# paulffm/Continuous-Time-Diffusion-Models-for-Discrete-Data

Measured on AMD Instinct MI355X. Metric: tau-leaping sample-steps/s, higher is better.
Workload: dtype bf16; 1 GPU; MNIST tauLDR U-Net TauL step (config_tauUnet_mnist: D=784, S=256, 1000-step grid); batch_per_gpu=256, global_batch=256, D=784, S=256, parallelism=sample-sharded x1, no collective in the loop

## Files before the change

continuous-time-diffusion-models-for-discrete-data_amd/csrc/unet_resblock_kernels.hip:

```cpp
#include "row_tile.hpp"
#include "../../include/ctdd_unet.h"

namespace ctdd {
namespace {

constexpr int RB_THREADS = 256, RB_N = 192, RB_PST = 20, RB_MAXC = 384;

struct RbLds {
  int raw, slab, part, red, scale, total;
  int rsA, rs2, prows;
};
__host__ __device__ inline RbLds rb_layout(int H, int W, int C) {
  RbLds L;
  L.rsA = C * 2 + 32;
  L.rs2 = RB_N * 2 + 32;
  L.prows = (H + 2) * (W + 2);
  const int slabA = L.prows * L.rsA, slab2 = L.prows * L.rs2;
  L.raw = 0;
  L.slab = H * W * L.rsA;
  L.part = L.slab + (slabA > slab2 ? slabA : slab2);
  L.red = L.part + RB_THREADS * RB_PST * 4;
  L.scale = L.red + 2 * RB_MAXC * 8;
  L.total = L.scale + 2 * RB_MAXC * 4;
  return L;
// ... 128 lines not shown
  auto step = [&](u32x4 (&slot)[3][2], bf16x8 (&xf)[NPT][2], bf16x8 (&xnext)[NPT][2], int ci, auto guard) {
    constexpr bool GUARD = decltype(guard)::value;
    if (GUARD && ci >= nchunks) return;
    xload(xnext, ci + 1);
#pragma unroll
    for (int s = 0; s < 2; ++s)
#pragma unroll
      for (int t = 0; t < 3; ++t)
#pragma unroll
        for (int pt = 0; pt < NPT; ++pt)
          acc[t][pt] = __builtin_amdgcn_mfma_f32_16x16x32_bf16(__builtin_bit_cast(bf16x8, slot[t][s]), xf[pt][s], acc[t][pt], 0, 0, 0);
    if (!GUARD || ci + PD < nchunks) wload(slot, ci + PD);
  };
  static_assert(PD % 2 == 0, "the two pixel-fragment buffers alternate inside a group");
  bf16x8 xq[2][NPT][2];
  xload(xq[0], 0);
  int ci0 = 0;
  for (; ci0 + 2 * PD <= nchunks; ci0 += PD) {
#pragma unroll
    for (int u = 0; u < PD; ++u) step(wr[u], xq[u & 1], xq[(u + 1) & 1], ci0 + u, std::false_type{});
  }
  for (; ci0 < nchunks; ci0 += PD) {
#pragma unroll
    for (int u = 0; u < PD; ++u) step(wr[u], xq[u & 1], xq[(u + 1) & 1], ci0 + u, std::true_type{});
  }
}

template <int NPT>
__global__ __launch_bounds__(RB_THREADS, 1) void k_resblock_small(const ctdd_resblock_args a) {
  extern __shared__ __attribute__((aligned(16))) unsigned char sm[];
  constexpr int PD = 6;
  const int t = threadIdx.x, b = blockIdx.x;
  const int H = a.H, W = a.W, HW = H * W, C = a.C1 + a.C2, Wp = W + 2;
  const RbLds L = rb_layout(H, W, C);
  const int lane = t & 63, wv = t >> 6, lj = lane & 15, lq = lane >> 4;

  const int K1 = 9 * C, K2 = 9 * RB_N + (a.skip ? C : 0);
  const unsigned short* w1p = (const unsigned short*)a.w1 + (size_t)wv * (K1 / 64) * 3072 + lane * 8;
  const unsigned short* w2p = (const unsigned short*)a.w2 + (size_t)wv * (K2 / 64) * 3072 + lane * 8;
  u32x4 wr[PD][3][2];

  {
    const int noct = C >> 3, nvec = HW * noct;
    const unsigned short* s1 = (const unsigned short*)a.s1_bf16 + (size_t)b * HW * a.C1;
    const unsigned short* s2 = (const unsigned short*)a.s2_bf16 + (size_t)b * HW * a.C2;
    constexpr int MAXV = 12;
    u32x4 u[MAXV];
#pragma unroll
    for (int k = 0; k < MAXV; ++k) {
      const int v = t + k * RB_THREADS, p = v / noct, c0 = (v - p * noct) * 8;
      const unsigned short* src = c0 < a.C1 ? s1 + (size_t)p * a.C1 + c0 : s2 + (size_t)p * a.C2 + (c0 - a.C1);
      u[k] = v < nvec ? *(const u32x4*)src : (u32x4){0u, 0u, 0u, 0u};
    }
    rb_wprologue<PD>(wr, w1p);
#pragma unroll
    for (int k = 0; k < MAXV; ++k) {
      const int v = t + k * RB_THREADS, p = v / noct, c0 = (v - p * noct) * 8;
      if (v < nvec) *(u32x4*)(sm + L.raw + p * L.rsA + c0 * 2) = u[k];
    }
    const int nz = (L.part - L.slab) >> 4;
    for (int v = t; v < nz; v += RB_THREADS) *(uint4*)(sm + L.slab + v * 16) = make_uint4(0, 0, 0, 0);
    __syncthreads();
    rb_groupnorm(sm, L, L.raw, L.rsA, false, L.slab, L.rsA, HW, W, Wp, C, a.G1, a.gamma1, a.beta1, a.eps1);
  }

  int pix[NPT], prow[NPT], b3[NPT], b1[NPT];
#pragma unroll
  for (int pt = 0; pt < NPT; ++pt) {
    if constexpr (NPT == 1) {
      const int pe = lj < HW ? lj : HW - 1;
      pix[pt] = lj < HW ? lj : -1;
      prow[pt] = rb_prow(pe, W, Wp);
      b1[pt] = L.raw + pe * L.rsA + lq * 16;
    } else {
      const RbPix q = rb_tile_pixel(pt, lj, H, W);
      pix[pt] = q.ok ? q.p : -1;
      prow[pt] = q.row;
      b1[pt] = L.raw + q.p * L.rsA + lq * 16;
    }
    b3[pt] = L.slab + prow[pt] * L.rsA + lq * 16;
  }
  const int n0 = wv * 48;
  f32x4 acc[3][NPT];
#pragma unroll
  for (int tt = 0; tt < 3; ++tt)
#pragma unroll
    for (int pt = 0; pt < NPT; ++pt) acc[tt][pt] = (f32x4){0.0f, 0.0f, 0.0f, 0.0f};

  rb_gemm<NPT, PD>(acc, wr, w1p, K1 / 64, K1 / 64, C / 64, sm, b3, L.rsA, Wp, b1);
  __syncthreads();
  rb_wprologue<PD>(wr, w2p);
  {
    const int npc = L.rs2 >> 4, nv = L.prows * npc;
    for (int v = t; v < nv; v += RB_THREADS) {
      const int row = v / npc, y = row / Wp, x = row - y * Wp;
      if (y == 0 || y == H + 1 || x == 0 || x == W + 1) *(uint4*)(sm + L.slab + v * 16) = make_uint4(0, 0, 0, 0);
    }
#pragma unroll
    for (int tt = 0; tt < 3; ++tt) {
      const int n = n0 + tt * 16 + lq * 4;
      const float4 bv = *(const float4*)(a.bias1 + n);
      const float4 tb = a.tbias ? *(const float4*)(a.tbias + (size_t)b * a.tb_stride + n) : make_float4(0.0f, 0.0f, 0.0f, 0.0f);
      const float add[4] = {bv.x + tb.x, bv.y + tb.y, bv.z + tb.z, bv.w + tb.w};
#pragma unroll
      for (int pt = 0; pt < NPT; ++pt) {
        if (pix[pt] >= 0) {
          const f32x4 v = acc[tt][pt];
          *(uint2*)(sm + L.slab + prow[pt] * L.rs2 + n * 2) =
              make_uint2(rt_pack2(v[0] + add[0], v[1] + add[1]), rt_pack2(v[2] + add[2], v[3] + add[3]));
        }
        acc[tt][pt] = (f32x4){0.0f, 0.0f, 0.0f, 0.0f};
      }
    }
  }
  __syncthreads();

  rb_groupnorm(sm, L, L.slab, L.rs2, true, L.slab, L.rs2, HW, W, Wp, RB_N, a.G2, a.gamma2, a.beta2, a.eps2);

#pragma unroll
  for (int pt = 0; pt < NPT; ++pt) b3[pt] = L.slab + prow[pt] * L.rs2 + lq * 16;
  rb_gemm<NPT, PD>(acc, wr, w2p, K2 / 64, 9 * RB_N / 64, RB_N / 64, sm, b3, L.rs2, Wp, b1);
  __syncthreads();
#pragma unroll
  for (int tt = 0; tt < 3; ++tt) {
    const int n = n0 + tt * 16 + lq * 4;
    const float4 bv = *(const float4*)(a.bias2 + n);
#pragma unroll
    for (int pt = 0; pt < NPT; ++pt) {
      if (pix[pt] >= 0) {
        const f32x4 v = acc[tt][pt];
        float o[4] = {v[0] + bv.x, v[1] + bv.y, v[2] + bv.z, v[3] + bv.w};
        if (!a.skip) {
          const uint2 r = *(const uint2*)(sm + L.raw + pix[pt] * L.rsA + n * 2);
          o[0] += __uint_as_float(r.x << 16); o[1] += __uint_as_float(r.x & 0xFFFF0000u);
          o[2] += __uint_as_float(r.y << 16); o[3] += __uint_as_float(r.y & 0xFFFF0000u);
        }
        *(uint2*)(sm + L.slab + pix[pt] * L.rs2 + n * 2) = make_uint2(rt_pack2(o[0], o[1]), rt_pack2(o[2], o[3]));
      }
    }
  }
  __syncthreads();
  {
    constexpr int npc = RB_N / 8;
    unsigned short* out = (unsigned short*)a.out_bf16 + (size_t)b * HW * RB_N;
    for (int v = t; v < HW * npc; v += RB_THREADS) {
      const int p = v / npc, c0 = (v - p * npc) * 8;
      *(uint4*)(out + (size_t)p * RB_N + c0) = *(const uint4*)(sm + L.slab + p * L.rs2 + c0 * 2);
    }
  }
}

constexpr int RM_NPT = 14, RM_PITCH = 16, RM_MAXH = 14, RM_MAXCS = 192;
constexpr int RM_RS = RB_N * 2 + 32;

__host__ __device__ inline RbLds rm_layout(int H, int W) {
  RbLds L;
  (void)W;
  L.rsA = L.rs2 = RB_N * 2 + 32;
  L.prows = (H + 2) * RM_PITCH;
  L.raw = L.slab = L.rs2;
  L.part = (L.prows + 2) * L.rs2;
  L.red = L.part + RB_THREADS * RB_PST * 4;
  L.scale = L.red + 2 * RB_MAXC * 8;
  L.total = L.scale + 2 * RB_MAXC * 4;
  return L;
}

__device__ __attribute__((always_inline)) inline void rm_gn1_stats(unsigned char* sm, const RbLds& L, const unsigned short* __restrict__ s1,
                                                                  const unsigned short* __restrict__ s2, int C1, int C2, int HW, int G,
                                                                  const float* __restrict__ gamma, const float* __restrict__ beta, float eps) {
  const int t = threadIdx.x, C = C1 + C2, noct = C >> 3;
  const int npl = RB_THREADS / noct < HW ? RB_THREADS / noct : HW, T = noct * npl;
  const bool act = t < T;
  const int oct = act ? t % noct : 0, pl = act ? t / noct : 0, c0 = oct * 8;
  const bool first = c0 < C1;
  const unsigned short* src = first ? s1 + c0 : s2 + (c0 - C1);
  const int cs = first ? C1 : C2;
  float* part = (float*)(sm + L.part);
  double* red = (double*)(sm + L.red);
  float* scale = (float*)(sm + L.scale);
  float* shift = scale + RB_MAXC;
  float sx[8], sq[8];
#pragma unroll
  for (int j = 0; j < 8; ++j) { sx[j] = 0.0f; sq[j] = 0.0f; }
  if (act) {
#pragma unroll 4
    for (int p = pl; p < HW; p += npl) {
      const u32x4 u = *(const u32x4*)(src + (size_t)p * cs);
#pragma unroll
      for (int j = 0; j < 4; ++j) {
        const float x0 = __uint_as_float(u[j] << 16), x1 = __uint_as_float(u[j] & 0xFFFF0000u);
        sx[2 * j] += x0; sq[2 * j] = fmaf(x0, x0, sq[2 * j]);
        sx[2 * j + 1] += x1; sq[2 * j + 1] = fmaf(x1, x1, sq[2 * j + 1]);
      }
    }
    float4* pt = (float4*)(part + t * RB_PST);
    pt[0] = make_float4(sx[0], sx[1], sx[2], sx[3]); pt[1] = make_float4(sx[4], sx[5], sx[6], sx[7]);
    pt[2] = make_float4(sq[0], sq[1], sq[2], sq[3]); pt[3] = make_float4(sq[4], sq[5], sq[6], sq[7]);
  }
  __syncthreads();
  for (int r = t; r < 2 * C; r += RB_THREADS) {
    const int m = r >= C ? 1 : 0, c = r - m * C;
    const float* pp = part + (c >> 3) * RB_PST + m * 8 + (c & 7);
    double acc = 0.0;
    for (int q = 0; q < npl; ++q) acc += (double)pp[q * noct * RB_PST];
    red[r] = acc;
  }
  __syncthreads();
  const int cg = C / G;
  for (int c = t; c < C; c += RB_THREADS) {
    const int g0 = (c / cg) * cg;
    double s = 0.0, q = 0.0;
    for (int j = g0; j < g0 + cg; ++j) { s += red[j]; q += red[C + j]; }
    const double n = (double)cg * (double)HW;
    const double mean = s / n;
    const double var = fmax(q / n - mean * mean, 0.0);
    const float rstd = (float)(1.0 / sqrt(var + (double)eps));
    scale[c] = rstd * gamma[c];
    shift[c] = beta[c] - (float)mean * rstd * gamma[c];
  }
  __syncthreads();
}

__device__ __attribute__((always_inline)) inline void rm_gn1_apply(unsigned char* sm, const RbLds& L, const unsigned short* __restrict__ src, int cs,
                                                                  int coff, int HW, int W) {
  const int t = threadIdx.x, noct = cs >> 3, npl = RB_THREADS / noct;
  if (t >= noct * npl) return;
  const int oct = t % noct, pl = t / noct;
  const float* scale = (const float*)(sm + L.scale) + coff + oct * 8;
  const float* shift = scale + RB_MAXC;
  const float4 sc0 = *(const float4*)scale, sc1 = *(const float4*)(scale + 4);
  const float4 sh0 = *(const float4*)shift, sh1 = *(const float4*)(shift + 4);
  const f32x2v scv[4] = {{sc0.x, sc0.y}, {sc0.z, sc0.w}, {sc1.x, sc1.y}, {sc1.z, sc1.w}};
  const f32x2v shv[4] = {{sh0.x, sh0.y}, {sh0.z, sh0.w}, {sh1.x, sh1.y}, {sh1.z, sh1.w}};
  const unsigned short* sp = src + oct * 8;
#pragma unroll 4
  for (int p = pl; p < HW; p += npl) {
    const u32x4 u = *(const u32x4*)(sp + (size_t)p * cs);
    unsigned ow[4];
#pragma unroll
    for (int j = 0; j < 4; ++j) {
      const f32x2v x = {__uint_as_float(u[j] << 16), __uint_as_float(u[j] & 0xFFFF0000u)};
      f32x2v y = __builtin_elementwise_fma(x, scv[j], shv[j]);
      const f32x2v z = y * (f32x2v){-1.4426950408889634f, -1.4426950408889634f};
      const f32x2v d = (f32x2v){__builtin_amdgcn_exp2f(z.x), __builtin_amdgcn_exp2f(z.y)} + (f32x2v){1.0f, 1.0f};
      y = y * (f32x2v){__builtin_amdgcn_rcpf(d.x), __builtin_amdgcn_rcpf(d.y)};
      ow[j] = rt_pack2(y.x, y.y);
    }
    *(uint4*)(sm + L.slab + rb_prow(p, W, RM_PITCH) * L.rs2 + oct * 16) = make_uint4(ow[0], ow[1], ow[2], ow[3]);
  }
}

__device__ __attribute__((always_inline)) inline void rm_wprologue(u32x4 (&wr)[2][3][3], const unsigned short* __restrict__ wrow, int nunits) {
#pragma unroll
  for (int u = 0; u < 2; ++u)
    if (u < nunits) rt_wload9(wr[u], wrow, u);
}

template <bool FULL>
__device__ __attribute__((always_inline)) inline void rm_gemm_skip(f32x4 (&acc)[3][RM_NPT], u32x4 (&ws)[2][3], const unsigned short* __restrict__ wrow, int nsk,
                                                                  const unsigned short* __restrict__ s1, const unsigned short* __restrict__ s2,
                                                                  int C1, int C2, int xc, int lq, int H, int W) {
  const int nc1 = C1 >> 5;
  auto gload = [&](bf16x8 (&g)[RM_NPT], int u) {
    const int ue = u < nsk ? u : nsk - 1;
    const bool two = ue >= nc1;
    const unsigned char* base = (const unsigned char*)(two ? s2 : s1);
    const int cs = two ? C2 : C1, cb = (ue - (two ? nc1 : 0)) * 32 + lq * 8;
#pragma unroll
    for (int y = 0; y < RM_NPT; ++y) {
      const int ye = FULL || y < H ? y : H - 1;
      g[y] = *(const bf16x8*)(base + (unsigned)(((ye * W + xc) * cs + cb) * 2));
    }
  };
  auto step = [&](u32x4 (&slot)[3], bf16x8 (&gc)[RM_NPT], bf16x8 (&gn)[RM_NPT], int u, auto guard) {
    constexpr bool GUARD = decltype(guard)::value;
    if (GUARD && u >= nsk) return;
    gload(gn, u + 1);
#pragma unroll
    for (int y = 0; y < RM_NPT; ++y) {
      if (FULL || y < H) {
#pragma unroll
        for (int t = 0; t < 3; ++t)
          acc[t][y] = __builtin_amdgcn_mfma_f32_16x16x32_bf16(__builtin_bit_cast(bf16x8, slot[t]), gc[y], acc[t][y], 0, 0, 0);
      }
    }
    if (!GUARD || u + 2 < nsk) rt_wload3(slot, wrow, u + 2);
    __builtin_amdgcn_sched_barrier(0);
  };
  bf16x8 G[2][RM_NPT];
  gload(G[0], 0);
  __builtin_amdgcn_s_waitcnt(0x0F70);
  int u0 = 0;
  for (; u0 + 4 <= nsk; u0 += 2) {
    step(ws[0], G[0], G[1], u0, std::false_type{});
    step(ws[1], G[1], G[0], u0 + 1, std::false_type{});
  }
  for (; u0 < nsk; u0 += 2) {
    step(ws[0], G[0], G[1], u0, std::true_type{});
    step(ws[1], G[1], G[0], u0 + 1, std::true_type{});
  }
}

template <bool FULL>
__global__ __launch_bounds__(RB_THREADS, 1) void k_resblock_mid(const ctdd_resblock_args a) {
  extern __shared__ __attribute__((aligned(16))) unsigned char sm[];
  constexpr int NPT = RM_NPT;
  const int t = threadIdx.x, b = blockIdx.x;
  const int H = FULL ? RM_NPT : a.H, W = a.W, HW = H * W, C1 = a.C1, C2 = a.C2;
  const RbLds L = rm_layout(H, W);
  const int lane = t & 63, wv = t >> 6, lj = lane & 15, lq = lane >> 4;
  const int nu1a = 3 * (C1 >> 5), nu1b = 3 * (C2 >> 5), nsk = a.skip ? (C1 + C2) >> 5 : 0;
  const unsigned short* w1p = (const unsigned short*)a.w1 + (size_t)wv * (nu1a + nu1b) * RT_UNIT + lane * 8;
  const unsigned short* s1 = (const unsigned short*)a.s1_bf16 + (size_t)b * HW * C1;
  const unsigned short* s2 = (const unsigned short*)a.s2_bf16 + (size_t)b * HW * C2;
  u32x4 wr[2][3][3];

  rm_wprologue(wr, w1p, nu1a);
  for (int v = t; v < (L.part >> 4); v += RB_THREADS) *(uint4*)(sm + v * 16) = make_uint4(0, 0, 0, 0);
  rm_gn1_stats(sm, L, s1, s2, C1, C2, HW, a.G1, a.gamma1, a.beta1, a.eps1);

  const int fb = L.slab + lj * RM_RS + lq * 16;
  const int n0 = wv * 48;
  f32x4 acc[3][NPT];
#pragma unroll
  for (int tt = 0; tt < 3; ++tt)
#pragma unroll
    for (int pt = 0; pt < NPT; ++pt) acc[tt][pt] = (f32x4){0.0f, 0.0f, 0.0f, 0.0f};

  for (int s = 0; s < (C2 ? 2 : 1); ++s) {
    rm_gn1_apply(sm, L, s ? s2 : s1, s ? C2 : C1, s ? C1 : 0, HW, W);
    __syncthreads();
    rt_gemm_rows<FULL, RM_RS, RM_PITCH>(acc, wr, w1p + (size_t)(s ? nu1a : 0) * RT_UNIT, s ? nu1b : nu1a, sm, fb, H);
    __syncthreads();
    if (s == 0 && C2) rm_wprologue(wr, w1p + (size_t)nu1a * RT_UNIT, nu1b);
  }
  const int tw = rt_again(t);
  const unsigned short* w2p = (const unsigned short*)a.w2 + (size_t)(tw >> 6) * (18 * RT_UNIT + nsk * 1536) + (tw & 63) * 8;
  u32x4 ws[2][3];
  if (nsk) {
    rt_wload3(ws[0], w2p + (size_t)18 * RT_UNIT, 0);
    if (nsk > 1) rt_wload3(ws[1], w2p + (size_t)18 * RT_UNIT, 1);
  } else {
    rm_wprologue(wr, w2p, 18);
  }
  const int lj1 = rt_again(lj);
  const bool own1 = lj1 >= 1 && lj1 <= W;
#pragma unroll
  for (int tt = 0; tt < 3; ++tt) {
    const int n = n0 + tt * 16 + lq * 4;
    const float4 bv = *(const float4*)(a.bias1 + n);
    const float4 tb = a.tbias ? *(const float4*)(a.tbias + (size_t)b * a.tb_stride + n) : make_float4(0.0f, 0.0f, 0.0f, 0.0f);
    const float add[4] = {bv.x + tb.x, bv.y + tb.y, bv.z + tb.z, bv.w + tb.w};
#pragma unroll
    for (int y = 0; y < NPT; ++y) {
      if (y < H && own1) {
        const f32x4 v = acc[tt][y];
        *(uint2*)(sm + L.slab + ((y + 1) * RM_PITCH + lj1) * RM_RS + n * 2) =
            make_uint2(rt_pack2(v[0] + add[0], v[1] + add[1]), rt_pack2(v[2] + add[2], v[3] + add[3]));
      }
      acc[tt][y] = (f32x4){0.0f, 0.0f, 0.0f, 0.0f};
    }
  }
  __syncthreads();

  if (nsk) {
    const int ljs = rt_again(lj), xc = ljs < 1 ? 0 : (ljs > W ? W - 1 : ljs - 1);
    rm_gemm_skip<FULL>(acc, ws, w2p + (size_t)18 * RT_UNIT, nsk, s1, s2, C1, C2, xc, lq, H, W);
    rm_wprologue(wr, w2p, 18);
  }

  rb_groupnorm(sm, L, L.slab, L.rs2, true, L.slab, L.rs2, HW, W, RM_PITCH, RB_N, a.G2, a.gamma2, a.beta2, a.eps2);
  rt_gemm_rows<FULL, RM_RS, RM_PITCH>(acc, wr, w2p, 18, sm, fb, H);
  __syncthreads();
  const int lj2 = rt_again(lj);
  const bool own2 = lj2 >= 1 && lj2 <= W;
  const int x2 = own2 ? lj2 - 1 : 0;
#pragma unroll
  for (int tt = 0; tt < 3; ++tt) {
    const int n = n0 + tt * 16 + lq * 4;
    const float4 bv = *(const float4*)(a.bias2 + n);
    uint2 r[NPT] = {};
    if (!a.skip) {
#pragma unroll
      for (int y = 0; y < NPT; ++y) r[y] = *(const uint2*)(s1 + (size_t)((y < H ? y : H - 1) * W + x2) * RB_N + n);
    }
#pragma unroll
    for (int y = 0; y < NPT; ++y) {
      if (y < H && own2) {
        const f32x4 v = acc[tt][y];
        float o[4] = {v[0] + bv.x, v[1] + bv.y, v[2] + bv.z, v[3] + bv.w};
        if (!a.skip) {
          o[0] += __uint_as_float(r[y].x << 16); o[1] += __uint_as_float(r[y].x & 0xFFFF0000u);
          o[2] += __uint_as_float(r[y].y << 16); o[3] += __uint_as_float(r[y].y & 0xFFFF0000u);
        }
        *(uint2*)(sm + L.slab + (y * W + x2) * RM_RS + n * 2) = make_uint2(rt_pack2(o[0], o[1]), rt_pack2(o[2], o[3]));
      }
    }
  }
  __syncthreads();
  {
    constexpr int npc = RB_N / 8;
    unsigned short* out = (unsigned short*)a.out_bf16 + (size_t)b * HW * RB_N;
    for (int v = t; v < HW * npc; v += RB_THREADS) {
      const int p = v / npc, c0 = (v - p * npc) * 8;
      *(uint4*)(out + (size_t)p * RB_N + c0) = *(const uint4*)(sm + L.slab + p * RM_RS + c0 * 2);
    }
  }
}

}
}

using namespace ctdd;

extern "C" int ctdd_unet_resblock_small(const void* args_, int f32, void* stream) {
  CTDD_REQUIRE(args_, CTDD_EINVAL, "ctdd_unet_resblock_small: null arguments");
  const ctdd_resblock_args& a = *(const ctdd_resblock_args*)args_;
  CTDD_REQUIRE(f32 == 0, CTDD_ERANGE, "ctdd_unet_resblock_small: bf16 inference only (the fp32 mode keeps the four launches)");
  const int span = (a.H - 1) * (a.W + 2) + a.W;
  CTDD_REQUIRE(a.B > 0 && a.H > 0 && a.W > 0 && a.W <= 8 && a.H * a.W <= 64 && (a.H * a.W <= 16 || span <= 80), CTDD_ERANGE,
               "ctdd_unet_resblock_small: a sample of %dx%d pixels does not fit the workgroup tile (H*W <= 64, W <= 8, (H-1)(W+2)+W <= 80)", a.H, a.W);
  const int C = a.C1 + a.C2;
  CTDD_REQUIRE(a.N == RB_N && a.C1 > 0 && a.C1 % 64 == 0 && a.C2 >= 0 && a.C2 % 64 == 0 && C <= RB_MAXC, CTDD_ERANGE,
               "ctdd_unet_resblock_small: channel counts off the tile (N=%d, C1=%d, C2=%d; N = 192, sources in multiples of 64, <= 384)", a.N,
               a.C1, a.C2);
  CTDD_REQUIRE(a.G1 > 0 && C % a.G1 == 0 && a.G2 > 0 && RB_N % a.G2 == 0, CTDD_EINVAL, "ctdd_unet_resblock_small: groups do not divide the channels");
  CTDD_REQUIRE(a.skip || (a.C2 == 0 && a.C1 == RB_N), CTDD_EINVAL, "ctdd_unet_resblock_small: a residual block needs C1 == N and one source");
  CTDD_REQUIRE(a.s1_bf16 && (a.C2 == 0 || a.s2_bf16) && a.w1 && a.w2 && a.bias1 && a.bias2 && a.gamma1 && a.beta1 && a.gamma2 && a.beta2 &&
                   a.out_bf16, CTDD_EINVAL, "ctdd_unet_resblock_small: null pointer");
  const RbLds L = rb_layout(a.H, a.W, C);
  CTDD_REQUIRE(L.total <= 160 * 1024, CTDD_ERANGE, "ctdd_unet_resblock_small: LDS image of %d bytes over the 160 KiB budget", L.total);
  hipStream_t st = (hipStream_t)stream;
  static bool attr_done[3][16] = {};
  if (a.H * a.W <= 16) {
    ensure_lds_ceiling((const void*)k_resblock_small<1>, attr_done[0]);
    hipLaunchKernelGGL(k_resblock_small<1>, dim3(a.B), dim3(RB_THREADS), (size_t)L.total, st, a);
  } else if (span > 64) {
    ensure_lds_ceiling((const void*)k_resblock_small<5>, attr_done[2]);
    hipLaunchKernelGGL(k_resblock_small<5>, dim3(a.B), dim3(RB_THREADS), (size_t)L.total, st, a);
  } else {
    ensure_lds_ceiling((const void*)k_resblock_small<4>, attr_done[1]);
    hipLaunchKernelGGL(k_resblock_small<4>, dim3(a.B), dim3(RB_THREADS), (size_t)L.total, st, a);
  }
  return finish_launch("k_resblock_small");
}

extern "C" int ctdd_unet_resblock_mid(const void* args_, int f32, void* stream) {
  CTDD_REQUIRE(args_, CTDD_EINVAL, "ctdd_unet_resblock_mid: null arguments");
  const ctdd_resblock_args& a = *(const ctdd_resblock_args*)args_;
  CTDD_REQUIRE(f32 == 0, CTDD_ERANGE, "ctdd_unet_resblock_mid: bf16 inference only (the fp32 mode keeps the four launches)");
  CTDD_REQUIRE(a.B > 0 && a.H > 0 && a.W > 0 && a.H <= RM_MAXH && a.W <= RM_PITCH - 2, CTDD_ERANGE,
               "ctdd_unet_resblock_mid: a sample of %dx%d pixels does not fit the workgroup tile (H <= 14, W <= 14)", a.H, a.W);
  const int C = a.C1 + a.C2;
  CTDD_REQUIRE(a.N == RB_N && a.C1 > 0 && a.C1 % 32 == 0 && a.C1 <= RM_MAXCS && a.C2 >= 0 && a.C2 % 32 == 0 && a.C2 <= RM_MAXCS, CTDD_ERANGE,
               "ctdd_unet_resblock_mid: channel counts off the tile (N=%d, C1=%d, C2=%d; N = 192, sources in multiples of 32, <= 192 each)", a.N,
               a.C1, a.C2);
  CTDD_REQUIRE(a.G1 > 0 && C % a.G1 == 0 && a.G2 > 0 && RB_N % a.G2 == 0, CTDD_EINVAL, "ctdd_unet_resblock_mid: groups do not divide the channels");
  CTDD_REQUIRE(a.skip || (a.C2 == 0 && a.C1 == RB_N), CTDD_EINVAL, "ctdd_unet_resblock_mid: a residual block needs C1 == N and one source");
  CTDD_REQUIRE(a.s1_bf16 && (a.C2 == 0 || a.s2_bf16) && a.w1 && a.w2 && a.bias1 && a.bias2 && a.gamma1 && a.beta1 && a.gamma2 && a.beta2 &&
                   a.out_bf16, CTDD_EINVAL, "ctdd_unet_resblock_mid: null pointer");
  const RbLds L = rm_layout(a.H, a.W);
  CTDD_REQUIRE(L.total <= 160 * 1024, CTDD_ERANGE, "ctdd_unet_resblock_mid: LDS image of %d bytes over the 160 KiB budget", L.total);
  static bool attr_done[2][16] = {};
  if (a.H == RM_NPT) {
    ensure_lds_ceiling((const void*)k_resblock_mid<true>, attr_done[1]);
    hipLaunchKernelGGL(k_resblock_mid<true>, dim3(a.B), dim3(RB_THREADS), (size_t)L.total, (hipStream_t)stream, a);
  } else {
    ensure_lds_ceiling((const void*)k_resblock_mid<false>, attr_done[0]);
    hipLaunchKernelGGL(k_resblock_mid<false>, dim3(a.B), dim3(RB_THREADS), (size_t)L.total, (hipStream_t)stream, a);
  }
  return finish_launch("k_resblock_mid");
}
```

continuous-time-diffusion-models-for-discrete-data_amd/csrc/unet_rows_kernels.hip:

```cpp
#include "row_tile.hpp"
#include "../../include/ctdd_unet.h"

namespace ctdd {
namespace {

constexpr int CR_N = 96, CR_BAND = 14, CR_PITCH = 32, CR_RS = 224, CR_MAXW = 28, CR_MAXC = 384, CR_PIECE = 96;
constexpr int CR_SLAB = ((CR_BAND + 2) * CR_PITCH + 2) * CR_RS;
constexpr int CR_SCALE = CR_SLAB;
constexpr int CR_RED = CR_SCALE + 2 * CR_MAXC * 4;
constexpr int CR_TOTAL = CR_RED + 2 * CR_N * 2 * 8;
constexpr int CR_FB = 12;
constexpr int CR_CARRY = CR_BAND * CR_MAXW * CR_RS;
static_assert(CR_CARRY + 4 * 3 * 2 * 64 * 16 <= CR_SLAB, "the output image and the upper waves' partial sums reuse the slab");

template <int THREADS, int FB>
__device__ __attribute__((always_inline)) inline void cr_fill(unsigned char* sm, const unsigned short* __restrict__ src, int cs, int pc, int coff,
                                                             int y0, int H, int W) {
  const int t = threadIdx.x, noct = pc >> 3, npl = THREADS / noct;
  if (t >= noct * npl) return;
  const int oct = t % noct, pl = t / noct;
  const float* scale = (const float*)(sm + CR_SCALE) + coff + oct * 8;
  const float* shift = scale + CR_MAXC;
  const float4 sc0 = *(const float4*)scale, sc1 = *(const float4*)(scale + 4);
  const float4 sh0 = *(const float4*)shift, sh1 = *(const float4*)(shift + 4);
  const f32x2v scv[4] = {{sc0.x, sc0.y}, {sc0.z, sc0.w}, {sc1.x, sc1.y}, {sc1.z, sc1.w}};
  const f32x2v shv[4] = {{sh0.x, sh0.y}, {sh0.z, sh0.w}, {sh1.x, sh1.y}, {sh1.z, sh1.w}};
  const int rlo = y0 == 0 ? 1 : 0, rhi = H - y0 < CR_BAND + 1 ? H - y0 : CR_BAND + 1;
  const unsigned npix = (unsigned)((rhi - rlo + 1) * W), uW = (unsigned)W;
  const unsigned short* sp = src + (size_t)((y0 - 1 + rlo) * W) * cs + oct * 8;
  unsigned char* dst = sm + (1 + rlo * CR_PITCH + 1) * CR_RS + oct * 16;
  for (unsigned p0 = (unsigned)pl; p0 < npix; p0 += (unsigned)(FB * npl)) {
    u32x4 u[FB];
#pragma unroll
    for (int k = 0; k < FB; ++k) {
      const unsigned p = p0 + (unsigned)(k * npl);
      u[k] = *(const u32x4*)(sp + (size_t)(p < npix ? p : npix - 1) * cs);
    }
#pragma unroll
    for (int k = 0; k < FB; ++k) {
      const unsigned p = p0 + (unsigned)(k * npl);
      unsigned ow[4];
#pragma unroll
      for (int j = 0; j < 4; ++j) {
        const f32x2v x = {__uint_as_float(u[k][j] << 16), __uint_as_float(u[k][j] & 0xFFFF0000u)};
        f32x2v y = __builtin_elementwise_fma(x, scv[j], shv[j]);
        const f32x2v z = y * (f32x2v){-1.4426950408889634f, -1.4426950408889634f};
        const f32x2v d = (f32x2v){__builtin_amdgcn_exp2f(z.x), __builtin_amdgcn_exp2f(z.y)} + (f32x2v){1.0f, 1.0f};
        y = y * (f32x2v){__builtin_amdgcn_rcpf(d.x), __builtin_amdgcn_rcpf(d.y)};
        ow[j] = rt_pack2(y.x, y.y);
      }
      const unsigned rr = p / uW, x = p - rr * uW;
      if (p < npix) *(uint4*)(dst + (rr * CR_PITCH + x) * CR_RS) = make_uint4(ow[0], ow[1], ow[2], ow[3]);
    }
  }
}

template <int NPT>
__device__ __attribute__((always_inline)) inline void cr_gemm_skip(f32x4 (&acc)[3][NPT], u32x4 (&ws)[2][3], const unsigned short* __restrict__ wrow, int nsk,
                                                                  const unsigned short* __restrict__ r1, const unsigned short* __restrict__ r2,
                                                                  int C1, int C2, int xc, int lq, int y0, int H, int W) {
  const int nc1 = C1 >> 5;
  auto gload = [&](bf16x8 (&g)[NPT], int u) {
    const int ue = u < nsk ? u : nsk - 1;
    const bool two = ue >= nc1;
    const unsigned char* base = (const unsigned char*)(two ? r2 : r1);
    const int cs = two ? C2 : C1, cb = (ue - (two ? nc1 : 0)) * 32 + lq * 8;
#pragma unroll
    for (int y = 0; y < NPT; ++y) {
      const int ye = y0 + y < H ? y0 + y : H - 1;
      g[y] = *(const bf16x8*)(base + (unsigned)(((ye * W + xc) * cs + cb) * 2));
    }
  };
  auto step = [&](u32x4 (&slot)[3], bf16x8 (&gc)[NPT], bf16x8 (&gn)[NPT], int u, auto guard) {
    constexpr bool GUARD = decltype(guard)::value;
    if (GUARD && u >= nsk) return;
    gload(gn, u + 1);
#pragma unroll
    for (int y = 0; y < NPT; ++y)
#pragma unroll
      for (int t = 0; t < 3; ++t)
        acc[t][y] = __builtin_amdgcn_mfma_f32_16x16x32_bf16(__builtin_bit_cast(bf16x8, slot[t]), gc[y], acc[t][y], 0, 0, 0);
    if (!GUARD || u + 2 < nsk) rt_wload3(slot, wrow, u + 2);
    __builtin_amdgcn_sched_barrier(0);
  };
  bf16x8 G[2][NPT];
  gload(G[0], 0);
  __builtin_amdgcn_s_waitcnt(0x0F70);
  int u0 = 0;
  for (; u0 + 4 <= nsk; u0 += 2) {
    step(ws[0], G[0], G[1], u0, std::false_type{});
    step(ws[1], G[1], G[0], u0 + 1, std::false_type{});
  }
  for (; u0 < nsk; u0 += 2) {
    step(ws[0], G[0], G[1], u0, std::true_type{});
    step(ws[1], G[1], G[0], u0 + 1, std::true_type{});
  }
}

#ifdef CTDD_ROWS_STAMPS
#define CR_STAMP(i_)                                                                                      \
  do {                                                                                                    \
    unsigned long long t_;                                                                                \
    asm volatile("s_memtime %0\n\ts_waitcnt lgkmcnt(0)" : "=s"(t_)::"memory");                            \
    if (threadIdx.x == 0) ((unsigned long long*)a.out_stats)[(size_t)blockIdx.x * 8 + (i_)] = t_;         \
  } while (0)
#else
#define CR_STAMP(i_)
#endif

template <bool SKIP, int WAVES>
__global__ __launch_bounds__(WAVES * 64, 1) void k_conv_rows(const ctdd_conv_rows_args a) {
  static_assert(WAVES == 4 || WAVES == 8, "one or two row halves");
  constexpr int CR_THREADS = WAVES * 64, NPT = CR_BAND * 4 / WAVES;
  extern __shared__ __attribute__((aligned(16))) unsigned char sm[];
  const int t = threadIdx.x;
  const int H = a.H, W = a.W, HW = H * W, C1 = a.C1, C2 = a.C2, C = C1 + C2;
  const int nbands = (H + CR_BAND - 1) / CR_BAND;
  const int b = blockIdx.x / nbands, y0 = (blockIdx.x - b * nbands) * CR_BAND;
  const int lane = t & 63, wv = t >> 6, lj = lane & 15, lq = lane >> 4, cg = WAVES == 8 ? (wv >> 1) & 1 : wv >> 1, hh = wv & 1;
  const int rh = WAVES == 8 ? __builtin_amdgcn_readfirstlane(wv >> 2) : 0, yw = y0 + NPT * rh;
  const int nu3 = 3 * (C >> 5), nsk = SKIP ? (a.RC1 + a.RC2) >> 5 : 0;
  const unsigned short* wrow = (const unsigned short*)a.w + (size_t)cg * ((size_t)nu3 * RT_UNIT + (size_t)nsk * 1536) + lane * 8;
  u32x4 wr[2][3][3];
  CR_STAMP(0);

  rt_wload9(wr[0], wrow, 0);
  rt_wload9(wr[1], wrow, 1);
  for (int v = t; v < (CR_SLAB >> 4); v += CR_THREADS) *(uint4*)(sm + v * 16) = make_uint4(0, 0, 0, 0);
  {
    float* scale = (float*)(sm + CR_SCALE);
    float* shift = scale + CR_MAXC;
    const int cgp = C / a.G;
    for (int c = t; c < C; c += CR_THREADS) {
      const int g0 = (c / cgp) * cgp;
      double s = 0.0, q = 0.0;
      for (int j = g0; j < g0 + cgp; ++j) {
        const double* st = j < C1 ? a.st1 + ((size_t)b * C1 + j) * 2 : a.st2 + ((size_t)b * C2 + (j - C1)) * 2;
        s += st[0]; q += st[1];
      }
      const double n = (double)cgp * (double)HW;
      const double mean = s / n;
      const double var = fmax(q / n - mean * mean, 0.0);
      const float rstd = (float)(1.0 / sqrt(var + (double)a.eps));
      scale[c] = rstd * a.gamma[c];
      shift[c] = a.beta[c] - (float)mean * rstd * a.gamma[c];
    }
  }
  __syncthreads();
  CR_STAMP(1);

  const int fb = (1 + 16 * hh + lj) * CR_RS + lq * 16 + rh * (NPT * CR_PITCH * CR_RS);
  f32x4 acc[3][NPT];
#pragma unroll
  for (int tt = 0; tt < 3; ++tt)
#pragma unroll
    for (int y = 0; y < NPT; ++y) acc[tt][y] = (f32x4){0.0f, 0.0f, 0.0f, 0.0f};

  int ub = 0;
  for (int s = 0; s < (C2 ? 2 : 1); ++s) {
    const int cs = s ? C2 : C1, coff = s ? C1 : 0;
    const unsigned short* src = (const unsigned short*)(s ? a.s2_bf16 : a.s1_bf16) + (size_t)b * HW * cs;
    for (int c0 = 0; c0 < cs; c0 += CR_PIECE) {
      const int pc = cs - c0 < CR_PIECE ? cs - c0 : CR_PIECE, nun = 3 * (pc >> 5);
      cr_fill<CR_THREADS, CR_FB * 4 / WAVES>(sm, src + c0, cs, pc, coff + c0, y0, H, W);
      __syncthreads();
      if constexpr (WAVES == 8)
        rt_gemm_rows_1buf<CR_RS, CR_PITCH>(acc, wr, wrow + (size_t)ub * RT_UNIT, nun, sm, fb);
      else
        rt_gemm_rows<true, CR_RS, CR_PITCH>(acc, wr, wrow + (size_t)ub * RT_UNIT, nun, sm, fb, NPT);
      __syncthreads();
      ub += nun;
      if (ub < nu3) {
        rt_wload9(wr[0], wrow + (size_t)ub * RT_UNIT, 0);
        rt_wload9(wr[1], wrow + (size_t)ub * RT_UNIT, 1);
      }
    }
  }
  CR_STAMP(2);

  if constexpr (SKIP) {
    const unsigned short* wsk = wrow + (size_t)nu3 * RT_UNIT;
    u32x4 ws[2][3];
    rt_wload3(ws[0], wsk, 0);
    if (nsk > 1) rt_wload3(ws[1], wsk, 1);
    const int cs_ = 16 * hh + rt_again(lj), xc = cs_ < 1 ? 0 : (cs_ > W ? W - 1 : cs_ - 1);
    cr_gemm_skip(acc, ws, wsk, nsk, (const unsigned short*)a.r1_bf16 + (size_t)b * HW * a.RC1,
                 (const unsigned short*)a.r2_bf16 + (size_t)b * HW * a.RC2, a.RC1, a.RC2, xc, lq, yw, H, W);
  }
  CR_STAMP(3);

  const int col = 16 * hh + rt_again(lj);
  const bool own = col >= 1 && col <= W;
  const int x2 = own ? col - 1 : 0;
  const int nrows = H - y0 < CR_BAND ? H - y0 : CR_BAND;
  const int nr = WAVES == 8 ? (nrows - NPT * rh < 0 ? 0 : (nrows - NPT * rh < NPT ? nrows - NPT * rh : NPT)) : nrows;
  double* red = (double*)(sm + CR_RED);
  float4* carry = (float4*)(sm + CR_CARRY) + (wv & 3) * (3 * 2 * 64) + lane;
  uint2 rr[3][NPT] = {};
  const bool res = !SKIP && a.res_bf16;
  if (res) {
    const unsigned short* rp = (const unsigned short*)a.res_bf16 + (size_t)b * HW * CR_N + cg * 48 + lq * 4;
#pragma unroll
    for (int y = 0; y < NPT; ++y) {
      const unsigned short* rpy = rp + (size_t)(((y < nr ? yw + y : H - 1)) * W + x2) * CR_N;
#pragma unroll
      for (int tt = 0; tt < 3; ++tt) rr[tt][y] = *(const uint2*)(rpy + tt * 16);
    }
  }
#pragma unroll
  for (int tt = 0; tt < 3; ++tt) {
    const int n = cg * 48 + tt * 16 + lq * 4;
    const float4 bv = *(const float4*)(a.bias + n);
    const float4 tb = a.tbias ? *(const float4*)(a.tbias + (size_t)b * a.tb_stride + n) : make_float4(0.0f, 0.0f, 0.0f, 0.0f);
    const float add[4] = {bv.x + tb.x, bv.y + tb.y, bv.z + tb.z, bv.w + tb.w};
    const uint2 (&r)[NPT] = rr[tt];
    float s[4] = {0.0f, 0.0f, 0.0f, 0.0f}, q[4] = {0.0f, 0.0f, 0.0f, 0.0f};
#pragma unroll
    for (int y = 0; y < NPT; ++y) {
      if (y < nr && own) {
        const f32x4 v = acc[tt][y];
        float o[4] = {v[0] + add[0], v[1] + add[1], v[2] + add[2], v[3] + add[3]};
        if (res) {
          o[0] += __uint_as_float(r[y].x << 16); o[1] += __uint_as_float(r[y].x & 0xFFFF0000u);
          o[2] += __uint_as_float(r[y].y << 16); o[3] += __uint_as_float(r[y].y & 0xFFFF0000u);
        }
        if (WAVES == 8 && rh) {
          acc[tt][y] = (f32x4){o[0], o[1], o[2], o[3]};
        } else {
#pragma unroll
          for (int i = 0; i < 4; ++i) { s[i] += o[i]; q[i] = fmaf(o[i], o[i], q[i]); }
        }
        *(uint2*)(sm + ((NPT * rh + y) * W + x2) * CR_RS + n * 2) = make_uint2(rt_pack2(o[0], o[1]), rt_pack2(o[2], o[3]));
      }
    }
#ifndef CTDD_ROWS_STAMPS
    if (a.out_stats) {
      if constexpr (WAVES == 4) {
#pragma unroll
        for (int i = 0; i < 4; ++i) {
          double ds = (double)s[i], dq = (double)q[i];
#pragma unroll
          for (int m = 1; m < 16; m <<= 1) { ds += __shfl_xor(ds, m, WAVE); dq += __shfl_xor(dq, m, WAVE); }
          if (lj == 0) { red[(hh * CR_N + n + i) * 2] = ds; red[(hh * CR_N + n + i) * 2 + 1] = dq; }
        }
      } else if (!rh) {
        carry[(tt * 2) * 64] = make_float4(s[0], s[1], s[2], s[3]);
        carry[(tt * 2 + 1) * 64] = make_float4(q[0], q[1], q[2], q[3]);
      }
    }
#endif
  }
  __syncthreads();
  CR_STAMP(4);
#ifndef CTDD_ROWS_STAMPS
  if (WAVES == 8 && rh && a.out_stats) {
#pragma unroll
    for (int tt = 0; tt < 3; ++tt) {
      const float4 cs_ = carry[(tt * 2) * 64], cq = carry[(tt * 2 + 1) * 64];
      float s[4] = {cs_.x, cs_.y, cs_.z, cs_.w}, q[4] = {cq.x, cq.y, cq.z, cq.w};
#pragma unroll
      for (int y = 0; y < NPT; ++y) {
        if (y < nr && own) {
#pragma unroll
          for (int i = 0; i < 4; ++i) { s[i] += acc[tt][y][i]; q[i] = fmaf(acc[tt][y][i], acc[tt][y][i], q[i]); }
        }
      }
      const int n = cg * 48 + tt * 16 + lq * 4;
#pragma unroll
      for (int i = 0; i < 4; ++i) {
        double ds = (double)s[i], dq = (double)q[i];
#pragma unroll
        for (int m = 1; m < 16; m <<= 1) { ds += __shfl_xor(ds, m, WAVE); dq += __shfl_xor(dq, m, WAVE); }
        if (lj == 0) { red[(hh * CR_N + n + i) * 2] = ds; red[(hh * CR_N + n + i) * 2 + 1] = dq; }
      }
    }
  }
#endif
  {
    constexpr int npc = CR_N / 8;
    unsigned short* out = (unsigned short*)a.out_bf16 + ((size_t)b * HW + (size_t)y0 * W) * CR_N;
    for (int v = t; v < nrows * W * npc; v += CR_THREADS) {
      const int p = v / npc, c0 = (v - p * npc) * 8;
      *(uint4*)(out + (size_t)p * CR_N + c0) = *(const uint4*)(sm + p * CR_RS + c0 * 2);
    }
#ifndef CTDD_ROWS_STAMPS
    if (WAVES == 8) __syncthreads();
    if (a.out_stats && t < 2 * CR_N) atomicAdd(a.out_stats + (size_t)b * CR_N * 2 + t, red[t] + red[2 * CR_N + t]);
#endif
  }
  CR_STAMP(5);
}

}
}

using namespace ctdd;

template <int WAVES>
static int launch_conv_rows(const void* args_, int f32, void* stream) {
  CTDD_REQUIRE(args_, CTDD_EINVAL, "ctdd_unet_conv_rows: null arguments");
  const ctdd_conv_rows_args& a = *(const ctdd_conv_rows_args*)args_;
  CTDD_REQUIRE(f32 == 0, CTDD_ERANGE, "ctdd_unet_conv_rows: bf16 inference only (the fp32 mode keeps GroupNorm and convolution apart)");
  CTDD_REQUIRE(a.B > 0 && a.H > 0 && a.W >= 1 && a.W <= CR_MAXW, CTDD_ERANGE,
               "ctdd_unet_conv_rows: a grid of %dx%d pixels does not fit the row tiles (1 <= W <= 28)", a.H, a.W);
  const int nbands = (a.H + CR_BAND - 1) / CR_BAND;
  CTDD_REQUIRE((int64_t)a.B * nbands < ((int64_t)1 << 31) && (int64_t)a.H * a.W * CR_MAXC < ((int64_t)1 << 30), CTDD_ERANGE,
               "ctdd_unet_conv_rows: B=%d, %dx%d is over the 32-bit index range of the kernel", a.B, a.H, a.W);
  const int C = a.C1 + a.C2;
  CTDD_REQUIRE(a.N == CR_N && a.C1 > 0 && a.C1 % 32 == 0 && a.C2 >= 0 && a.C2 % 32 == 0 && C <= CR_MAXC && a.RC1 >= 0 && a.RC1 % 32 == 0 &&
                   a.RC2 >= 0 && a.RC2 % 32 == 0 && (a.RC2 == 0 || a.RC1 > 0) && a.RC1 + a.RC2 <= CR_MAXC, CTDD_ERANGE,
               "ctdd_unet_conv_rows: channel counts off the tile (N=%d, C1=%d, C2=%d, RC1=%d, RC2=%d; N = 96, sources in multiples of 32, <= 384 in all)",
               a.N, a.C1, a.C2, a.RC1, a.RC2);
  CTDD_REQUIRE(a.G > 0 && C % a.G == 0, CTDD_EINVAL, "ctdd_unet_conv_rows: %d groups do not divide %d channels", a.G, C);
  CTDD_REQUIRE(a.s1_bf16 && (a.C2 == 0 || a.s2_bf16) && (a.RC1 == 0 || a.r1_bf16) && (a.RC2 == 0 || a.r2_bf16) && a.gamma && a.beta && a.w &&
                   a.bias && a.out_bf16, CTDD_EINVAL, "ctdd_unet_conv_rows: null pointer");
  CTDD_REQUIRE(a.st1 && (a.C2 == 0 || a.st2), CTDD_EINVAL, "ctdd_unet_conv_rows: a GroupNorm source without statistics");
  auto al16 = [](const void* p) { return ((uintptr_t)p & 15) == 0; };
  CTDD_REQUIRE(al16(a.s1_bf16) && al16(a.s2_bf16) && al16(a.r1_bf16) && al16(a.r2_bf16) && al16(a.res_bf16) && al16(a.w) && al16(a.out_bf16) &&
                   al16(a.bias) && al16(a.tbias) && a.tb_stride % 4 == 0, CTDD_EINVAL, "ctdd_unet_conv_rows: tensors must be 16-byte aligned");
  CTDD_REQUIRE(!(a.RC1 > 0 && a.res_bf16), CTDD_EINVAL, "ctdd_unet_conv_rows: 1x1 segments and a residual in one call");
  static bool attr_done[2][16] = {};
  if (a.RC1 > 0) {
    ensure_lds_ceiling((const void*)k_conv_rows<true, WAVES>, attr_done[1]);
    hipLaunchKernelGGL((k_conv_rows<true, WAVES>), dim3(a.B * nbands), dim3(WAVES * 64), (size_t)CR_TOTAL, (hipStream_t)stream, a);
  } else {
    ensure_lds_ceiling((const void*)k_conv_rows<false, WAVES>, attr_done[0]);
    hipLaunchKernelGGL((k_conv_rows<false, WAVES>), dim3(a.B * nbands), dim3(WAVES * 64), (size_t)CR_TOTAL, (hipStream_t)stream, a);
  }
  return finish_launch("k_conv_rows");
}

extern "C" int ctdd_unet_conv_rows(const void* args_, int f32, void* stream) { return launch_conv_rows<8>(args_, f32, stream); }
extern "C" int ctdd_unet_conv_rows_w4(const void* args_, int f32, void* stream) { return launch_conv_rows<4>(args_, f32, stream); }
```

Before: 138,500 sample-steps/s.

## Deepen skip-GEMM prefetch pipeline and batch GroupNorm stats loads

Replaces the double-buffered skip-connection GEMM in the mid and row resblock kernels with a D-deep (default 3) software pipeline that issues each next global activation load right after its MFMA, and keeps D weight slots in flight. GroupNorm-1 statistics now issue 20 loads at once before consuming them, with LDS zeroing overlapped between request and use. Also adds optional timestamp probes and hoists the bias loads. The deeper buffers raise register pressure in kernels launched at one block per CU, which risks spills.

```diff
diff --git a/continuous-time-diffusion-models-for-discrete-data_amd/csrc/unet_resblock_kernels.hip b/continuous-time-diffusion-models-for-discrete-data_amd/csrc/unet_resblock_kernels.hip
--- a/continuous-time-diffusion-models-for-discrete-data_amd/csrc/unet_resblock_kernels.hip
+++ b/continuous-time-diffusion-models-for-discrete-data_amd/csrc/unet_resblock_kernels.hip
@@ -304,6 +304,10 @@
 
 constexpr int RM_NPT = 14, RM_PITCH = 16, RM_MAXH = 14, RM_MAXCS = 192;
 constexpr int RM_RS = RB_N * 2 + 32;
+#ifndef CTDD_RM_SKIP_DEPTH
+#define CTDD_RM_SKIP_DEPTH 3
+#endif
+constexpr int RM_SKIP_DEPTH = CTDD_RM_SKIP_DEPTH;
 
 __host__ __device__ inline RbLds rm_layout(int H, int W) {
   RbLds L;
@@ -318,9 +322,11 @@
   return L;
 }
 
+constexpr int RM_FB = 20;
 __device__ __attribute__((always_inline)) inline void rm_gn1_stats(unsigned char* sm, const RbLds& L, const unsigned short* __restrict__ s1,
                                                                   const unsigned short* __restrict__ s2, int C1, int C2, int HW, int G,
-                                                                  const float* __restrict__ gamma, const float* __restrict__ beta, float eps) {
+                                                                  const float* __restrict__ gamma, const float* __restrict__ beta, float eps,
+                                                                  int nzero) {
   const int t = threadIdx.x, C = C1 + C2, noct = C >> 3;
   const int npl = RB_THREADS / noct < HW ? RB_THREADS / noct : HW, T = noct * npl;
   const bool act = t < T;
@@ -335,16 +341,34 @@
   float sx[8], sq[8];
 #pragma unroll
   for (int j = 0; j < 8; ++j) { sx[j] = 0.0f; sq[j] = 0.0f; }
+  u32x4 u[RM_FB];
+  auto request = [&](int p0) {
+#pragma unroll
+    for (int k = 0; k < RM_FB; ++k) {
+      const int p = p0 + k * npl;
+      if (p < HW) u[k] = *(const u32x4*)(src + (size_t)p * cs);
+    }
+  };
+  auto consume = [&](int p0) {
+#pragma unroll
+    for (int k = 0; k < RM_FB; ++k) {
+      if (p0 + k * npl < HW) {
+#pragma unroll
+        for (int j = 0; j < 4; ++j) {
+          const float x0 = __uint_as_float(u[k][j] << 16), x1 = __uint_as_float(u[k][j] & 0xFFFF0000u);
+          sx[2 * j] += x0; sq[2 * j] = fmaf(x0, x0, sq[2 * j]);
+          sx[2 * j + 1] += x1; sq[2 * j + 1] = fmaf(x1, x1, sq[2 * j + 1]);
+        }
+      }
+    }
+  };
+  if (act) request(pl);
+  for (int v = t; v < nzero; v += RB_THREADS) *(uint4*)(sm + v * 16) = make_uint4(0, 0, 0, 0);
   if (act) {
-#pragma unroll 4
-    for (int p = pl; p < HW; p += npl) {
-      const u32x4 u = *(const u32x4*)(src + (size_t)p * cs);
-#pragma unroll
-      for (int j = 0; j < 4; ++j) {
-        const float x0 = __uint_as_float(u[j] << 16), x1 = __uint_as_float(u[j] & 0xFFFF0000u);
-        sx[2 * j] += x0; sq[2 * j] = fmaf(x0, x0, sq[2 * j]);
-        sx[2 * j + 1] += x1; sq[2 * j + 1] = fmaf(x1, x1, sq[2 * j + 1]);
-      }
+    consume(pl);
+    for (int p0 = pl + RM_FB * npl; p0 < HW; p0 += RM_FB * npl) {
+      request(p0);
+      consume(p0);
     }
     float4* pt = (float4*)(part + t * RB_PST);
     pt[0] = make_float4(sx[0], sx[1], sx[2], sx[3]); pt[1] = make_float4(sx[4], sx[5], sx[6], sx[7]);
@@ -409,11 +433,59 @@
     if (u < nunits) rt_wload9(wr[u], wrow, u);
 }
 
-template <bool FULL>
-__device__ __attribute__((always_inline)) inline void rm_gemm_skip(f32x4 (&acc)[3][RM_NPT], u32x4 (&ws)[2][3], const unsigned short* __restrict__ wrow, int nsk,
-                                                                  const unsigned short* __restrict__ s1, const unsigned short* __restrict__ s2,
+template <bool FULL, int D>
+__device__ __attribute__((always_inline)) inline void rm_gemm_skip(f32x4 (&acc)[3][RM_NPT], u32x4 (&ws)[D == 1 ? 2 : D][3], const unsigned short* __restrict__ wrow,
+                                                                  int nsk, const unsigned short* __restrict__ s1, const unsigned short* __restrict__ s2,
                                                                   int C1, int C2, int xc, int lq, int H, int W) {
   const int nc1 = C1 >> 5;
+  if constexpr (D > 1) {
+    bf16x8 G[D][RM_NPT];
+    auto gload1 = [&](bf16x8& g, int u, int y) {
+      const bool two = u >= nc1;
+      const unsigned char* base = (const unsigned char*)(two ? s2 : s1);
+      const int cs = two ? C2 : C1, cb = (u - (two ? nc1 : 0)) * 32 + lq * 8;
+      const int ye = FULL || y < H ? y : H - 1;
+      g = *(const bf16x8*)(base + (unsigned)(((ye * W + rt_again(xc)) * cs + cb) * 2));
+    };
+    auto step = [&](u32x4 (&slot)[3], bf16x8 (&g)[RM_NPT], int u, auto guard) {
+      constexpr bool GUARD = decltype(guard)::value;
+      if (GUARD && u >= nsk) return;
+      const bool more = !GUARD || u + D < nsk;
+#pragma unroll
+      for (int y = 0; y < RM_NPT; ++y) {
+        if (FULL || y < H) {
+#pragma unroll
+          for (int t = 0; t < 3; ++t)
+            acc[t][y] = __builtin_amdgcn_mfma_f32_16x16x32_bf16(__builtin_bit_cast(bf16x8, slot[t]), g[y], acc[t][y], 0, 0, 0);
+          if (more) gload1(g[y], u + D, y);
+          __builtin_amdgcn_sched_barrier(0);
+        }
+      }
+      if (more) rt_wload3(slot, wrow, u + D);
+      __builtin_amdgcn_sched_barrier(0);
+    };
+#pragma unroll
+    for (int k = 0; k < D; ++k)
+      if (k < nsk) {
+#pragma unroll
+        for (int y = 0; y < RM_NPT; ++y) gload1(G[k][y], k, y);
+      }
+    __builtin_amdgcn_s_waitcnt(0x0F70);
+    int u0 = 0;
+    for (; u0 + 2 * D <= nsk; u0 += D) {
+#pragma unroll
+      for (int k = 0; k < D; ++k) step(ws[k], G[k], u0 + k, std::false_type{});
+    }
+#pragma unroll
+    for (int i = 0; i < 2; ++i) {
+      if (u0 < nsk) {
+#pragma unroll
+        for (int k = 0; k < D; ++k) step(ws[k], G[k], u0 + k, std::true_type{});
+        u0 += D;
+      }
+    }
+    return;
+  }
   auto gload = [&](bf16x8 (&g)[RM_NPT], int u) {
     const int ue = u < nsk ? u : nsk - 1;
     const bool two = ue >= nc1;
@@ -453,6 +525,18 @@
     step(ws[1], G[1], G[0], u0 + 1, std::true_type{});
   }
 }
+
+#ifdef CTDD_RESBLOCK_STAMPS
+#define RM_STAMP(i_)                                                                                                      \
+  do {                                                                                                                    \
+    unsigned long long t_;                                                                                                \
+    asm volatile("s_memtime %0\n\ts_waitcnt lgkmcnt(0)" : "=s"(t_)::"memory");                                            \
+    if (threadIdx.x == 0)                                                                                                 \
+      ((unsigned long long*)((unsigned short*)a.out_bf16 + (size_t)a.B * a.H * a.W * RB_N))[(size_t)blockIdx.x * 16 + (i_)] = t_; \
+  } while (0)
+#else
+#define RM_STAMP(i_)
+#endif
 
 template <bool FULL>
 __global__ __launch_bounds__(RB_THREADS, 1) void k_resblock_mid(const ctdd_resblock_args a) {
@@ -467,10 +551,11 @@
   const unsigned short* s1 = (const unsigned short*)a.s1_bf16 + (size_t)b * HW * C1;
   const unsigned short* s2 = (const unsigned short*)a.s2_bf16 + (size_t)b * HW * C2;
   u32x4 wr[2][3][3];
+  RM_STAMP(0);
 
   rm_wprologue(wr, w1p, nu1a);
-  for (int v = t; v < (L.part >> 4); v += RB_THREADS) *(uint4*)(sm + v * 16) = make_uint4(0, 0, 0, 0);
-  rm_gn1_stats(sm, L, s1, s2, C1, C2, HW, a.G1, a.gamma1, a.beta1, a.eps1);
+  rm_gn1_stats(sm, L, s1, s2, C1, C2, HW, a.G1, a.gamma1, a.beta1, a.eps1, L.part >> 4);
+  RM_STAMP(1);
 
   const int fb = L.slab + lj * RM_RS + lq * 16;
   const int n0 = wv * 48;
@@ -483,18 +568,23 @@
   for (int s = 0; s < (C2 ? 2 : 1); ++s) {
     rm_gn1_apply(sm, L, s ? s2 : s1, s ? C2 : C1, s ? C1 : 0, HW, W);
     __syncthreads();
+    RM_STAMP(2 + 2 * s);
     rt_gemm_rows<FULL, RM_RS, RM_PITCH>(acc, wr, w1p + (size_t)(s ? nu1a : 0) * RT_UNIT, s ? nu1b : nu1a, sm, fb, H);
     __syncthreads();
+    RM_STAMP(3 + 2 * s);
     if (s == 0 && C2) rm_wprologue(wr, w1p + (size_t)nu1a * RT_UNIT, nu1b);
   }
-  const int tw = rt_again(t);
-  const unsigned short* w2p = (const unsigned short*)a.w2 + (size_t)(tw >> 6) * (18 * RT_UNIT + nsk * 1536) + (tw & 63) * 8;
-  u32x4 ws[2][3];
+  auto w2ptr = [&]() {
+    const int tw = rt_again(t);
+    return (const unsigned short*)a.w2 + (size_t)(tw >> 6) * (18 * RT_UNIT + nsk * 1536) + (tw & 63) * 8;
+  };
+  u32x4 ws[RM_SKIP_DEPTH == 1 ? 2 : RM_SKIP_DEPTH][3];
   if (nsk) {
-    rt_wload3(ws[0], w2p + (size_t)18 * RT_UNIT, 0);
-    if (nsk > 1) rt_wload3(ws[1], w2p + (size_t)18 * RT_UNIT, 1);
+#pragma unroll
+    for (int k = 0; k < (RM_SKIP_DEPTH == 1 ? 2 : RM_SKIP_DEPTH); ++k)
+      if (k < nsk) rt_wload3(ws[k], w2ptr() + (size_t)18 * RT_UNIT, k);
   } else {
-    rm_wprologue(wr, w2p, 18);
+    rm_wprologue(wr, w2ptr(), 18);
   }
   const int lj1 = rt_again(lj);
   const bool own1 = lj1 >= 1 && lj1 <= W;
@@ -515,23 +605,30 @@
     }
   }
   __syncthreads();
+  RM_STAMP(6);
 
   if (nsk) {
     const int ljs = rt_again(lj), xc = ljs < 1 ? 0 : (ljs > W ? W - 1 : ljs - 1);
-    rm_gemm_skip<FULL>(acc, ws, w2p + (size_t)18 * RT_UNIT, nsk, s1, s2, C1, C2, xc, lq, H, W);
-    rm_wprologue(wr, w2p, 18);
-  }
-
-  rb_groupnorm(sm, L, L.slab, L.rs2, true, L.slab, L.rs2, HW, W, RM_PITCH, RB_N, a.G2, a.gamma2, a.beta2, a.eps2);
-  rt_gemm_rows<FULL, RM_RS, RM_PITCH>(acc, wr, w2p, 18, sm, fb, H);
-  __syncthreads();
-  const int lj2 = rt_again(lj);
+    rm_gemm_skip<FULL, RM_SKIP_DEPTH>(acc, ws, w2ptr() + (size_t)18 * RT_UNIT, nsk, s1, s2, C1, C2, xc, lq, H, W);
+    rm_wprologue(wr, w2ptr(), 18);
+  }
+  RM_STAMP(7);
+
+  rb_groupnorm(sm, L, L.slab, L.rs2, true, L.slab, L.rs2, rt_again(HW), W, RM_PITCH, RB_N, a.G2, a.gamma2, a.beta2, a.eps2);
+  RM_STAMP(8);
+  rt_gemm_rows<FULL, RM_RS, RM_PITCH>(acc, wr, w2ptr(), 18, sm, fb, H);
+  __syncthreads();
+  RM_STAMP(9);
+  const int t2 = rt_again(t), lj2 = t2 & 15, lq2 = (t2 >> 4) & 3, n2 = (t2 >> 6) * 48;
   const bool own2 = lj2 >= 1 && lj2 <= W;
   const int x2 = own2 ? lj2 - 1 : 0;
+  float4 bv2[3];
+#pragma unroll
+  for (int tt = 0; tt < 3; ++tt) bv2[tt] = *(const float4*)(a.bias2 + n2 + tt * 16 + lq2 * 4);
 #pragma unroll
   for (int tt = 0; tt < 3; ++tt) {
-    const int n = n0 + tt * 16 + lq * 4;
-    const float4 bv = *(const float4*)(a.bias2 + n);
+    const int n = n2 + tt * 16 + lq2 * 4;
+    const float4 bv = bv2[tt];
     uint2 r[NPT] = {};
     if (!a.skip) {
 #pragma unroll
@@ -551,6 +648,7 @@
     }
   }
   __syncthreads();
+  RM_STAMP(10);
   {
     constexpr int npc = RB_N / 8;
     unsigned short* out = (unsigned short*)a.out_bf16 + (size_t)b * HW * RB_N;
@@ -559,6 +657,7 @@
       *(uint4*)(out + (size_t)p * RB_N + c0) = *(const uint4*)(sm + L.slab + p * RM_RS + c0 * 2);
     }
   }
+  RM_STAMP(11);
 }
 
 }
diff --git a/continuous-time-diffusion-models-for-discrete-data_amd/csrc/unet_rows_kernels.hip b/continuous-time-diffusion-models-for-discrete-data_amd/csrc/unet_rows_kernels.hip
--- a/continuous-time-diffusion-models-for-discrete-data_amd/csrc/unet_rows_kernels.hip
+++ b/continuous-time-diffusion-models-for-discrete-data_amd/csrc/unet_rows_kernels.hip
@@ -10,6 +10,10 @@
 constexpr int CR_RED = CR_SCALE + 2 * CR_MAXC * 4;
 constexpr int CR_TOTAL = CR_RED + 2 * CR_N * 2 * 8;
 constexpr int CR_FB = 12;
+#ifndef CTDD_CR_SKIP_DEPTH
+#define CTDD_CR_SKIP_DEPTH 3
+#endif
+constexpr int CR_SKIP_DEPTH = CTDD_CR_SKIP_DEPTH;
 constexpr int CR_CARRY = CR_BAND * CR_MAXW * CR_RS;
 static_assert(CR_CARRY + 4 * 3 * 2 * 64 * 16 <= CR_SLAB, "the output image and the upper waves' partial sums reuse the slab");
 
@@ -55,11 +59,57 @@
   }
 }
 
-template <int NPT>
-__device__ __attribute__((always_inline)) inline void cr_gemm_skip(f32x4 (&acc)[3][NPT], u32x4 (&ws)[2][3], const unsigned short* __restrict__ wrow, int nsk,
-                                                                  const unsigned short* __restrict__ r1, const unsigned short* __restrict__ r2,
+template <int NPT, int D>
+__device__ __attribute__((always_inline)) inline void cr_gemm_skip(f32x4 (&acc)[3][NPT], u32x4 (&ws)[D == 1 ? 2 : D][3], const unsigned short* __restrict__ wrow,
+                                                                  int nsk, const unsigned short* __restrict__ r1, const unsigned short* __restrict__ r2,
                                                                   int C1, int C2, int xc, int lq, int y0, int H, int W) {
   const int nc1 = C1 >> 5;
+  if constexpr (D > 1) {
+    bf16x8 G[D][NPT];
+    auto gload1 = [&](bf16x8& g, int u, int y) {
+      const bool two = u >= nc1;
+      const unsigned char* base = (const unsigned char*)(two ? r2 : r1);
+      const int cs = two ? C2 : C1, cb = (u - (two ? nc1 : 0)) * 32 + lq * 8;
+      const int ye = y0 + y < H ? y0 + y : H - 1;
+      g = *(const bf16x8*)(base + (unsigned)(((ye * W + xc) * cs + cb) * 2));
+    };
+    auto step = [&](u32x4 (&slot)[3], bf16x8 (&g)[NPT], int u, auto guard) {
+      constexpr bool GUARD = decltype(guard)::value;
+      if (GUARD && u >= nsk) return;
+      const bool more = !GUARD || u + D < nsk;
+#pragma unroll
+      for (int y = 0; y < NPT; ++y) {
+#pragma unroll
+        for (int t = 0; t < 3; ++t)
+          acc[t][y] = __builtin_amdgcn_mfma_f32_16x16x32_bf16(__builtin_bit_cast(bf16x8, slot[t]), g[y], acc[t][y], 0, 0, 0);
+        if (more) gload1(g[y], u + D, y);
+        __builtin_amdgcn_sched_barrier(0);
+      }
+      if (more) rt_wload3(slot, wrow, u + D);
+      __builtin_amdgcn_sched_barrier(0);
+    };
+#pragma unroll
+    for (int k = 0; k < D; ++k)
+      if (k < nsk) {
+#pragma unroll
+        for (int y = 0; y < NPT; ++y) gload1(G[k][y], k, y);
+      }
+    __builtin_amdgcn_s_waitcnt(0x0F70);
+    int u0 = 0;
+    for (; u0 + 2 * D <= nsk; u0 += D) {
+#pragma unroll
+      for (int k = 0; k < D; ++k) step(ws[k], G[k], u0 + k, std::false_type{});
+    }
+#pragma unroll
+    for (int i = 0; i < 2; ++i) {
+      if (u0 < nsk) {
+#pragma unroll
+        for (int k = 0; k < D; ++k) step(ws[k], G[k], u0 + k, std::true_type{});
+        u0 += D;
+      }
+    }
+    return;
+  }
   auto gload = [&](bf16x8 (&g)[NPT], int u) {
     const int ue = u < nsk ? u : nsk - 1;
     const bool two = ue >= nc1;
@@ -180,12 +230,19 @@
 
   if constexpr (SKIP) {
     const unsigned short* wsk = wrow + (size_t)nu3 * RT_UNIT;
-    u32x4 ws[2][3];
+    constexpr int SD = WAVES == 8 ? CR_SKIP_DEPTH : 1;
+    u32x4 ws[SD == 1 ? 2 : SD][3];
     rt_wload3(ws[0], wsk, 0);
-    if (nsk > 1) rt_wload3(ws[1], wsk, 1);
+    if constexpr (SD == 1) {
+      if (nsk > 1) rt_wload3(ws[1], wsk, 1);
+    } else {
+#pragma unroll
+      for (int k = 1; k < SD; ++k)
+        if (k < nsk) rt_wload3(ws[k], wsk, k);
+    }
     const int cs_ = 16 * hh + rt_again(lj), xc = cs_ < 1 ? 0 : (cs_ > W ? W - 1 : cs_ - 1);
-    cr_gemm_skip(acc, ws, wsk, nsk, (const unsigned short*)a.r1_bf16 + (size_t)b * HW * a.RC1,
-                 (const unsigned short*)a.r2_bf16 + (size_t)b * HW * a.RC2, a.RC1, a.RC2, xc, lq, yw, H, W);
+    cr_gemm_skip<NPT, SD>(acc, ws, wsk, nsk, (const unsigned short*)a.r1_bf16 + (size_t)b * HW * a.RC1,
+                          (const unsigned short*)a.r2_bf16 + (size_t)b * HW * a.RC2, a.RC1, a.RC2, xc, lq, yw, H, W);
   }
   CR_STAMP(3);
 
```

Result: no change. 139,200 sample-steps/s, median of 6 (+0.5%).
